# andyljones/megastep

Hardware: AMD Instinct MI355X
Metric: env-steps/sec (higher is better)
Workload: dtype f32

## Files before the change

megastep_amd/_lib.py:

```python
import ctypes as C
import os
import subprocess
import torch

_HERE = os.path.dirname(os.path.abspath(__file__))
CSRC = os.path.join(_HERE, 'csrc')
LIB_PATH = os.environ.get('MEGASTEP_HIP_LIB') or os.path.join(CSRC, 'libmegastep_hip.so')
ABI_VERSION = 17

_f32p = C.POINTER(C.c_float)
_i32p = C.POINTER(C.c_int)


class MsConfig(C.Structure):
    _fields_ = [('agent_radius', C.c_float), ('res', C.c_int), ('fov', C.c_float), ('fps', C.c_float)]


class MsScenery(C.Structure):
    _fields_ = [
        ('n_envs', C.c_int), ('n_agents', C.c_int), ('n_model', C.c_int),
        ('lights_vals', C.c_void_p), ('lights_widths', C.c_void_p), ('lights_starts', C.c_void_p),
        ('lines_vals', C.c_void_p), ('lines_widths', C.c_void_p), ('lines_starts', C.c_void_p),
        ('lines_inverse', C.c_void_p),
        ('textures_vals', C.c_void_p), ('textures_widths', C.c_void_p), ('textures_starts', C.c_void_p),
# ... 139 lines not shown
    'ms_overhead': (_int, [_p(MsScenery), _p(MsAgents), _p(MsOverhead), _ptr]),
    'ms_nav_free': (_int, [_p(MsScenery), _p(MsNavGrid), _ptr]),
    'ms_nav_fields': (_int, [_p(MsNavGrid), _p(MsNavFields), _ptr]),
    'ms_nav_query': (_int, [_p(MsNavGrid), _p(MsNavQuery), _ptr]),
    'ms_nav_waypoints': (_int, [_p(MsNavGrid), _p(MsNavWaypoints), _ptr]),
    'ms_nav_paths': (_int, [_p(MsNavGrid), _p(MsNavPaths), _ptr]),
    'ms_nav_seen': (_int, [_p(MsNavGrid), _p(MsNavSeen), _ptr]),
    'ms_nav_windows': (_int, [_p(MsNavGrid), _p(MsNavWindows), _ptr]),
    'ms_nav_seed_fields': (_int, [_p(MsNavGrid), _p(MsNavSeedFields), _ptr]),
    'ms_nav_seed_waypoints': (_int, [_p(MsNavGrid), _p(MsNavSeedWaypoints), _ptr]),
    'ms_nav_seed_paths': (_int, [_p(MsNavGrid), _p(MsNavSeedPaths), _ptr]),
    'ms_wallgrid_scan': (_int, [_p(MsScenery), _p(MsWallGridParent), _ptr, _int, _int, _ptr, _ptr, _ptr, _ptr]),
    'ms_wallgrid_fill': (_int, [_p(MsScenery), _ptr, _int, _int, _ptr, _ptr, _ptr, _ptr, _ptr, _ptr]),
    'ms_host_ray_interval': (None, [_f32p, _f32p, _int, _flt, _flt, _int, _i32p, _i32p]),
    'ms_host_ray_interval_wide': (None, [_f32p, _f32p, _int, _flt, _flt, _int, _int, _i32p, _i32p]),
    'ms_debug_ray_groups': (_int, [_int]),
    'ms_debug_physics_pack': (_int, [_int]),
    'ms_debug_last_render_groups': (_int, []),
    'ms_debug_last_step_fused': (_int, []),
    'ms_host_render_plan': (C.c_longlong, [_int, _int, _int, _int, _int, _flt, _int, _i32p]),
    'ms_host_render_block': (_int, [_int, _int, _int, _int, _int, _flt, _int, C.c_longlong, _i32p]),
    'ms_host_physics_pack': (_int, [_int, _int, _int, _int]),
    'ms_debug_render_order': (_int, [_int]),
    'ms_host_order_fans': (_int, [_int, _i32p, _i32p]),
    'ms_debug_ray_group_tail': (_int, [_flt, _int]),
    'ms_debug_pair_telemetry': (_int, [_int]),
    'ms_debug_overhead_cull': (_int, [_int]),
    'ms_host_overhead_keeps': (_int, [_f32p, _int, _int, _int, _int, _flt, _f32p]),
    'ms_host_nav_waypoint': (_int, [_ptr, _flt, _ptr, _ptr, _ptr, _ptr, _int, _ptr]),
    'ms_host_nav_path': (_int, [_ptr, _flt, _ptr, _ptr, _ptr, _ptr, _int, _ptr]),
    'ms_host_nav_seed_field': (_int, [_ptr, _flt, _ptr, _ptr, _int, _ptr, _int, _ptr, _ptr]),
    'ms_host_nav_seed_waypoint': (_int, [_ptr, _flt, _ptr, _ptr, _ptr, _int, _ptr]),
    'ms_host_nav_seed_path': (_int, [_ptr, _flt, _ptr, _ptr, _ptr, _int, _ptr]),
    'ms_host_nav_seen': (_int, [_ptr, _flt, _ptr, _int, _int, _int, _ptr, _ptr, _ptr, _ptr, _flt, _ptr, _ptr, _ptr, _ptr]),
    'ms_host_nav_windows': (_int, [_p(MsNavGrid), _p(MsNavWindows)]),
    'ms_test_arithmetic': (_int, [_ptr]*7 + [C.c_longlong, _ptr]),
    'ms_host_lightgrid_cell': (_int, [_ptr, _int, _ptr, _int, _flt, _flt, _int, _int, _flt, _int, _ptr, _ptr, _int]),
    'ms_host_fold_hits': (_int, [_f32p, _i32p, _int, _i32p, _f32p, _i32p]),
    'ms_host_agents_apart': (_int, [_f32p, _f32p, _flt]),
    'ms_host_wall_beyond_reach': (_int, [_f32p, _f32p, _flt]),
    'ms_host_wall_reach': (_flt, [_f32p, _flt]),
    'ms_host_wall_hidden': (_int, [_flt]*4 + [_f32p, _f32p, _flt]),
    'ms_host_wall_sectors': (None, [_flt]*4 + [_f32p, _i32p, _i32p, _f32p, _i32p]),
    'ms_host_wallgrid_cell': (None, [_ptr, _int, _flt, _flt, _int, _int, _flt, _int, _flt, _flt, _flt, _ptr, _ptr]),
    'ms_host_wall_arc': (None, [_flt]*4 + [_f32p, _i32p, _i32p]),
    'ms_host_wedge_meets': (_int, [_flt]*4 + [_int, _int]),
# ... 100 lines not shown
```

megastep_amd/csrc/kernels/render.h:

```cpp
constexpr int PAIRS = 128;

struct Cand { float pqx, pqy, vx, vy; };

__device__ __attribute__((noinline)) float2 sincospi_called(const float x) {
    float s_, c_;
    sincospi_f(x, s_, c_);
    return make_float2(s_, c_);
}

__device__ inline float4 drawn_row(const float s, const float c, const float px, const float py, const float4 mdl) {
    float4 w;
    w.x = c*mdl.x - s*mdl.y + px; w.y = s*mdl.x + c*mdl.y + py;
    w.z = c*mdl.z - s*mdl.w + px; w.w = s*mdl.z + c*mdl.w + py;
    return w;
}
__device__ inline void camera_ray(const float cs, const float sn, const int r, const float Rf, const float half_screen,
                                  const float inv_res, float& rx, float& ry) {
    const float num = (Rf - 2*(float)r - 1)*half_screen;
    const float uy = inv_res != 0.f ? num*inv_res : div_inrange(num, Rf);
    rx = cs*1.f - sn*uy; ry = sn*1.f + cs*uy;
}
__host__ inline float camera_inv_res(const int R, const float half_screen) {
    return ((R & (R - 1)) == 0 && half_screen > 1e-3f) ? 1.f/(float)R : 0.f;
}
// ... 209 lines not shown
#define MS_AHEAD 1
#endif
#ifndef MS_VCAP
#define MS_VCAP 128
#endif
#ifndef MS_VCAP_WIDE
#define MS_VCAP_WIDE 110
#endif
#ifndef MS_WAVES_WIDE
#define MS_WAVES_WIDE 6
#endif
template <int OBS, int SHADE = 1, int NG = 1, int STEP = 0>
__global__ __launch_bounds__(WAVE) __attribute__((amdgpu_waves_per_eu(NG > 1 ? MS_WAVES_WIDE : MS_WAVES, NG > 1 ? MS_WAVES_WIDE : MS_WAVES))) void render_kernel(
        const MsScenery sc, const AgentsK ag, const MsRender out,
        const float agent_radius, const float half_screen, const int R, const int n_fans,
        const std::conditional_t<STEP == 1, RenderConstsStep, std::conditional_t<NG == 1, RenderConstsOrder, RenderConsts>> rc) {
    static_assert(STEP == 0 || NG == 1, "the fused step: one group of rays");
    constexpr bool ORDERED = NG == 1 && STEP == 0;
    PROBE_INIT
    static_assert(NG == 1 || NG == 2 || NG == 4, "one, two or four ray groups per wave");
    [[maybe_unused]] constexpr int NR = WAVE*NG;
    constexpr int VCAP = NG == 1 ? MS_VCAP : MS_VCAP_WIDE;
    constexpr int O_EPI = NG > 1 ? 24*VCAP + 256 : 0;
    constexpr int LDS_PER_WAVE = NG == 1 ? 24*VCAP + 3072 : O_EPI + 2816 + 6*VCAP;
    __shared__ __attribute__((aligned(16))) unsigned char s_raw[LDS_PER_WAVE];

    int lane = threadIdx.x;
#define LANE_AFRESH asm volatile("" : "+v"(lane))
    Cand* const s_cand_w = reinterpret_cast<Cand*>(&s_raw[0]);
    float* const s_screen_w = reinterpret_cast<float*>(&s_raw[O_EPI]);

    const int b = blockIdx.x;
    [[maybe_unused]] int fan = b;
    const int A = sc.n_agents, AF = sc.n_agents*sc.n_model;
    int n, a, r0, span;
    if constexpr (ORDERED) {
        const int slot = render_slot(b, n_fans);
        const int* const at = rc.schedule ? rc.schedule + n_fans + slot : sc.lines_starts;
        const int named = *at;
        fan = rc.schedule ? (int)min((unsigned)named, (unsigned)(n_fans - 1)) : slot;
        render_fan(fan, A, R, rc, n, a, r0, span);
    } else if (!render_block(b, n_fans, A, R, NG, rc, n, a, r0, span, fan)) return;
    const int r = r0 + lane;
    const int r_last = min(r0 + span - 1, R - 1);
    [[maybe_unused]] const int n_live = r_last - r0 + 1;

    const int L = sc.lines_widths[n];
// ... 177 lines not shown
    const float Rf = (float)R;
    auto ray_len = [&](const float rx_, const float ry_) {
        return sqrt_normal(rx_*rx_ + ry_*ry_);
    };
    auto ray_of = [&](const int r_, float& rx_, float& ry_, float& rlen_, float& near_) {
        camera_ray(cs, sn, r_, Rf, half_screen, rc.inv_res, rx_, ry_);
        rlen_ = ray_len(rx_, ry_);
        near_ = div_inrange(agent_radius, rlen_);
    };
    float rx, ry, rlen, near;
    ray_of(r, rx, ry, rlen, near);

    const float c_a = 0.5f*(Rf - 1.f), c_b = rc.c_b;
    const float x_clip = rc.x_clip;
    const float g0 = (float)r0;

    constexpr bool COLOUR = SHADE != 0;
    static_assert(COLOUR || OBS == 1, "without colour `screen` is NULL: the OBS instantiation");
    static_assert(OBS != 2 || (COLOUR && STEP == 0), "no per-ray planes at all: a colour instantiation");
    constexpr bool PLANES = OBS != 2;
    constexpr bool MASKED = !COLOUR || (OBS >= 1 && NG == 1);
    [[maybe_unused]] const int out_mask_ = MASKED ? (out.obs_subsample >> 8) : 0;
#define MS_WANTED(BIT, PTR) (MASKED ? ((out_mask_ & (BIT)) != 0) : ((PTR) != nullptr))
    [[maybe_unused]] int fan_cost = 0;
    auto winner_of = [&](const int nearest_idx, float4& hw_mem, int& tex_w, int& tstart) {
        const LateArgs late = late_args();
        const bool want_texel_row = COLOUR || (OBS && MS_WANTED(OUT_SEEN, late->out.seen_stamp));
        const bool want_line = want_texel_row || MS_WANTED(OUT_LOCATIONS, late->out.locations) || MS_WANTED(OUT_DOTS, late->out.dots);
        const int row = min(max(nearest_idx, 0), max(L - 1, 0));
        hw_mem = make_float4(0.f, 0.f, 0.f, 0.f); tex_w = 1; tstart = 0;
        if (want_line) hw_mem = rows.row(row);
        if (want_texel_row) {
            const int* const l_tex_widths = late->sc.textures_widths;
            const int* const l_tex_starts = late->sc.textures_starts;
            tex_w = l_tex_widths[base + row]; tstart = l_tex_starts[base + row];
        }
    };
    auto finish_group = [&](const int q, const int r, const float rx, const float ry, const float rlen,
                            const float nearest_s, const int nearest_idx, const float4 hw_mem, const int tex_w, const int tstart) {
    const LateArgs late = late_args();
    const bool want_texel_row = COLOUR || (OBS && MS_WANTED(OUT_SEEN, late->out.seen_stamp));
    const bool want_line = want_texel_row || MS_WANTED(OUT_LOCATIONS, late->out.locations) || MS_WANTED(OUT_DOTS, late->out.dots);
    float loc = NAN, dt = NAN;
    float4 hw = make_float4(0.f, 0.f, 0.f, 0.f);
    if (want_line) {
        float4 aw = make_float4(0.f, 0.f, 0.f, 0.f);
        if (__ballot((nearest_idx >= 0) & (nearest_idx < AF))) aw = agent_line(nearest_idx);
        if (nearest_idx >= 0) {
            hw = (nearest_idx < AF) ? aw : hw_mem;
            const float vx = hw.z - hw.x, vy = hw.w - hw.y;
            const float d = rx*vy - ry*vx;
            const float pqx = hw.x - pp.x, pqy = hw.y - pp.y;
            loc = div_inrange(pqx*ry - pqy*rx, d);
            const float dtop = rx*vx + ry*vy;
            const float dbot = rlen*sqrt_any(vx*vx + vy*vy);
            dt = div_inrange(dtop, dbot + 1.e-6f);
        }
    }
    [[maybe_unused]] const size_t o = ((size_t)n*A + a)*R + r;
    const float dist = nearest_s*rlen;
    if constexpr (PLANES) {
        if (!MASKED || (out_mask_ & (OUT_INDICES | OUT_LOCATIONS | OUT_DOTS | OUT_DISTANCES))) {
            int* const o_indices = late->out.indices;
            float* const o_locations = late->out.locations;
            float* const o_dots = late->out.dots;
            float* const o_distances = late->out.distances;
            if (r < R) {
                if (!OBS || MS_WANTED(OUT_INDICES, o_indices)) __builtin_nontemporal_store(nearest_idx, &o_indices[o]);
                if (!OBS || MS_WANTED(OUT_LOCATIONS, o_locations)) __builtin_nontemporal_store(loc, &o_locations[o]);
                if (!OBS || MS_WANTED(OUT_DOTS, o_dots)) __builtin_nontemporal_store(dt, &o_dots[o]);
                if (!OBS || MS_WANTED(OUT_DISTANCES, o_distances)) __builtin_nontemporal_store(dist, &o_distances[o]);
            }
        }
    }

// ... 120 lines not shown
        }
        for (int o2 = 4; o2 < sub; o2 <<= 1) {
            if constexpr (COLOUR) {
                p0 += __shfl_xor(p0, o2, WAVE); p1 += __shfl_xor(p1, o2, WAVE); p2 += __shfl_xor(p2, o2, WAVE);
            }
            pd += __shfl_xor(pd, o2, WAVE);
        }
        if (((lane & (sub - 1)) == 0) & (r < R)) {
            const int sh = __builtin_ctz((unsigned)sub);
            const float inv = bits_f((uint32_t)(127 - sh) << 23);
            const int W = R >> sh, px = r >> sh;
            const size_t na = (size_t)n*A + a;
            if (COLOUR && MS_WANTED(OUT_RGB, late->out.obs_rgb)) {
                late->out.obs_rgb[(na*3 + 0)*W + px] = p0*inv;
                late->out.obs_rgb[(na*3 + 1)*W + px] = p1*inv;
                late->out.obs_rgb[(na*3 + 2)*W + px] = p2*inv;
            }
            if (MS_WANTED(OUT_DEPTH, late->out.obs_depth)) late->out.obs_depth[na*W + px] = pd*inv;
        }
    }
    };
    float nearest_s = INFINITY;
    int nearest_idx = -1;

    constexpr int V_CAP = VCAP, P_CAP = 4096 < 64*VCAP ? 4096 : 64*VCAP;
    constexpr int O_INFO = 16*V_CAP;
    constexpr int O_QUEUE = NG == 1 ? 24*V_CAP + 768 : 24*V_CAP;
    constexpr int O_RAY = NG == 1 ? 24*V_CAP : O_EPI, O_NEAR = O_RAY + 512, O_BEST = NG == 1 ? O_QUEUE + 256 : O_NEAR + 256;
    constexpr int O_MARK = O_BEST + 1536, O_PINFO = O_MARK + 512, O_GK = O_PINFO + 4*V_CAP;
    static_assert((NG == 1 ? O_MARK + 512 : O_GK + 2*V_CAP) == LDS_PER_WAVE && LDS_PER_WAVE >= 2560, "the LDS block: lists, rays, queue, three key slots, 4096 mark bits");
    static_assert(NG == 1 || O_EPI + 2560 <= LDS_PER_WAVE, "the epilogue's scratch fits the per-group region");
    int2* const s_info_w = reinterpret_cast<int2*>(&s_raw[O_INFO]);
    float2* const s_ray_w = reinterpret_cast<float2*>(&s_raw[O_RAY]);
    float* const s_near_w = reinterpret_cast<float*>(&s_raw[O_NEAR]);
    unsigned long long* const s_best_w = reinterpret_cast<unsigned long long*>(&s_raw[O_BEST]);
    unsigned long long* const s_second_w = reinterpret_cast<unsigned long long*>(&s_raw[O_BEST + 512]);
    unsigned long long* const s_third_w = reinterpret_cast<unsigned long long*>(&s_raw[O_BEST + 1024]);
    unsigned* const s_mark_w = reinterpret_cast<unsigned*>(&s_raw[O_MARK]);
    if constexpr (NG == 1) {
        s_ray_w[lane] = make_float2(rx, ry);
        s_near_w[lane] = near;
        s_best_w[lane] = ~0ull;
        s_mark_w[lane] = 0u; s_mark_w[lane + WAVE] = 0u;
        s_second_w[lane] = ~0ull;
        s_third_w[lane] = ~0ull;
    }
    auto pseudo_angle_fast = [](const float x_, const float y_) {
        const float pq_ = y_*__builtin_amdgcn_rcpf(fabsf(x_) + fabsf(y_));
        return x_ < 0.f ? 2.f - pq_ : (pq_ < 0.f ? 4.f + pq_ : pq_);
    };
    const float pa_first = readlane_f(pseudo_angle_fast(rx, ry), 0);
    float pa_last = readlane_f(pseudo_angle_fast(rx, ry), min(n_live, WAVE) - 1);
    float sp_g0 = g0, sp_last = (float)(r_last - r0), sp_nr = (float)WAVE;
    auto fetch = [&](const int c0) { return rows.chunk(lane, c0); };
    auto line_math = [&](float4 w, const int l, const bool live, const bool agent_lines, const bool first_chunk, Cand& cd, int& lo, int& len) {
        if (agent_lines) {
            const float4 aw = agent_line_m(l, first_chunk, mdl_first);
            if (l < AF) w = aw;
        }
        const float pqx = w.x - pp.x, pqy = w.y - pp.y;
        const float dbx = w.z - pp.x, dby = w.w - pp.y;
// ... 39 lines not shown
                if (beyond) {
                    const unsigned long long key = ((unsigned long long)f_bits(sv) << 32) | (unsigned)info.y;
                    const unsigned long long old = atomicMin(&s_best_w[rr], key);
                    const unsigned oh = (unsigned)(old >> 32);
                    if (oh != 0xffffffffu) {
                        const bool won = key < old;
                        const float so = bits_f(oh);
                        const float front = won ? sv : so, back = won ? so : sv;
                        if (back < front + 4.e-4f) {
                            const unsigned long long lose1 = won ? old : key;
                            const unsigned long long old2 = atomicMin(&s_second_w[rr], lose1);
                            const unsigned long long lose2 = old2 > lose1 ? old2 : lose1;
                            if (lose2 != ~0ull) atomicMin(&s_third_w[rr], lose2);
                        }
                    }
                }
            }
        }
        __builtin_amdgcn_wave_barrier();
        s_mark_w[lane] = 0u; s_mark_w[lane + WAVE] = 0u;
        n_list = 0; n_pairs = 0;
    };

    auto admit = [&](const float4 w, const int l, const bool live, const bool agent_lines, const bool first_chunk) {
        Cand cd;
        int lo = 0, len = 0;
        line_math(w, l, live, agent_lines, first_chunk, cd, lo, len);
        const bool seen = len > 0;
        const unsigned long long vm = __ballot(seen);
        if (!vm) return;
        const int incl = wave_scan_add(len);
        const int chunk_pairs = __builtin_amdgcn_readlane(incl, 63);
        const int chunk_lines = __popcll(vm);
        if ((n_list + chunk_lines > V_CAP) | (n_pairs + chunk_pairs > P_CAP)) drain();
        if (seen) {
            const int k = n_list + (int)__builtin_amdgcn_mbcnt_hi((unsigned)(vm >> 32), __builtin_amdgcn_mbcnt_lo((unsigned)vm, 0u));
            const int first = n_pairs + incl - len;
            s_cand_w[k] = cd;
            s_info_w[k] = make_int2(lo - first, l);
            atomicOr(&s_mark_w[first >> 5], 1u << (first & 31));
        }
        n_list += chunk_lines; n_pairs += chunk_pairs;
    };

    constexpr int Q_CAP = 128;
    unsigned short* const s_queue_w = reinterpret_cast<unsigned short*>(&s_raw[O_QUEUE]);
    const bool listed = wg_count >= 0;
    const int n_raw = listed ? wg_count : max(L - AF, 0);
    const int own0 = a*sc.n_model, own = rc.skip_own ? sc.n_model : 0;
    const int AL = AF - own;
    const __amdgpu_buffer_rsrc_t list_rsrc = __builtin_amdgcn_make_buffer_rsrc(
        const_cast<unsigned*>(sc.wg_pool + wg_pool_base_n + wg_first), 0, listed ? 4*n_raw : 0, 0x00020000);
    auto raw = [&](const int k0) {
        return (unsigned)__builtin_amdgcn_raw_buffer_load_b32(list_rsrc, 4*(k0 + lane), 0, 0);
    };
    auto walk = [&](const float pa_right, const float pa_left, auto&& admit_fn, auto&& stop_fn) {
        int wa8, wb8;
        wg_wedge(pa_right, pa_left, wa8, wb8);
        unsigned e_next[2] = {raw(0), raw(WAVE)};
        int raw_pos = 0, q_len = 0, al_left = AL;
        int q_first = 0;
        for (;;) {
            while ((raw_pos < n_raw) & (q_len <= Q_CAP - WAVE)) {
                const unsigned e = e_next[0];
                e_next[0] = e_next[1];
                e_next[1] = raw(raw_pos + 2*WAVE);
                const int k = raw_pos + lane;
                const int idx = listed ? (int)(e & 0xffffu) : k;
                const bool keep = (k < n_raw) & (!listed | wg_arcs_meet((int)((e >> 16) & 255u), (int)(e >> 24), wa8, wb8));
                const unsigned long long km = __ballot(keep);
                if (keep) s_queue_w[q_len + (int)__builtin_amdgcn_mbcnt_hi((unsigned)(km >> 32), __builtin_amdgcn_mbcnt_lo((unsigned)km, 0u))] = (unsigned short)idx;
                q_len += __popcll(km);
                raw_pos += WAVE;
            }
            __builtin_amdgcn_fence(__ATOMIC_RELEASE, "wavefront");
            __builtin_amdgcn_wave_barrier();
            __builtin_amdgcn_fence(__ATOMIC_ACQUIRE, "wavefront");
            const int al0 = AL - al_left;
            const int n_al = min(al_left, AHEAD*WAVE);
            const int n_items = n_al + min(q_len, AHEAD*WAVE - n_al);
            const int q_used = n_items - n_al;
            int l_it[AHEAD];
            float4 w_it[AHEAD];
            #pragma unroll
            for (int kk = 0; kk < AHEAD; kk++) {
                const int i = kk*WAVE + lane;
                const int ai = al0 + i;
                const int q_at = min(max(i - n_al, 0), Q_CAP - 1);
                const int qe = listed ? (int)s_queue_w[q_at] : q_first + q_at;
                l_it[kk] = (i < n_al) ? ai + (ai >= own0 ? own : 0) : AF + qe;
                w_it[kk] = rows.load(l_it[kk]*16, 0);
            }
            PROBE_VAL(2, 0)
            PROBE_AT(3, w_it[0].x)
            #pragma unroll
            for (int kk = 0; kk < AHEAD; kk++) {
                if (kk*WAVE >= n_items) continue;
                admit_fn(w_it[kk], l_it[kk], kk*WAVE + lane < n_items, kk*WAVE < n_al, al0 + kk*WAVE == 0);
            }
            al_left -= n_al;
            __builtin_amdgcn_wave_barrier();
            if (q_used < q_len) {
                unsigned short keep_[Q_CAP/WAVE];
                #pragma unroll
                for (int j = 0; j < Q_CAP/WAVE; j++) keep_[j] = s_queue_w[min(q_used + j*WAVE + lane, Q_CAP - 1)];
                __builtin_amdgcn_wave_barrier();
                #pragma unroll
                for (int j = 0; j < Q_CAP/WAVE; j++) if (j*WAVE + lane < q_len - q_used) s_queue_w[j*WAVE + lane] = keep_[j];
            }
            q_len -= q_used;
            q_first += q_used;
            if (((raw_pos >= n_raw) & (q_len == 0) & (al_left == 0)) || stop_fn()) break;
        }
    };
    if constexpr (NG == 1) {
        walk(pa_last, pa_first, admit, [] { return false; });
        if (n_pairs) drain();
    }
    __builtin_amdgcn_fence(__ATOMIC_ACQUIRE, "wavefront");
    bool list_whole = true;
    auto resolve_group = [&](const int q, const float rx, const float ry, const float near, float& nearest_s, int& nearest_idx) {
        const unsigned long long best = s_best_w[lane], second = s_second_w[lane], third = s_third_w[lane];
        bool ambiguous = false;
        if (best != ~0ull) {
            const float s1 = bits_f((uint32_t)(best >> 32)), s2 = bits_f((uint32_t)(second >> 32)), s3 = bits_f((uint32_t)(third >> 32));
            const int i1 = (int)(uint32_t)best, i2 = (int)(uint32_t)second;
            nearest_s = s1;
            nearest_idx = i1;
            if ((second != ~0ull) && !(s1 < s2 - 1.e-4f)) {
                if ((third == ~0ull) || (s2 < s3 - 1.e-4f)) {
                    const bool first_is_1 = i1 < i2;
                    const float sa = first_is_1 ? s1 : s2, sb = first_is_1 ? s2 : s1;
                    const int ia = first_is_1 ? i1 : i2, ib = first_is_1 ? i2 : i1;
                    const bool b_wins = sb < sa - 1.e-4f;
                    nearest_s = b_wins ? sb : sa;
                    nearest_idx = b_wins ? ib : ia;
                } else {
                    ambiguous = true;
                }
            }
        }
        const unsigned long long amb = __ballot(ambiguous);
        if constexpr (ORDERED) fan_cost = n_windows + (list_n >> 5) + 4*(int)__popcll(amb);
        PROBE_VAL(11, n_pairs_total) PROBE_VAL(12, n_drains == 1 ? list_n : -1) PROBE_VAL(13, __popcll(amb))
#if MS_PROBE
        const unsigned t_fold0 = (unsigned)clock64();
        PROBE_VAL(15, t_fold0)
#endif
        if (out.workspace && lane == 0 && q == 0 && rc.telemetry) {
            atomicAdd(&out.workspace[3], n_pairs_total); atomicAdd(&out.workspace[4], n_windows);
        }
        if (amb && out.workspace && lane == 0) {
            atomicAdd(&out.workspace[1], __popcll(amb));
            if (__popcll(amb) > 6) atomicAdd(&out.workspace[2], 1);
        }
        if (amb && (NG == 1 ? n_drains == 1 : list_whole)) {
            const int rounds = (list_n + WAVE - 1)/WAVE;
            if (2*(int)__popcll(amb)*rounds <= list_n + 16) {
                float x = INFINITY;
                int xi = -1;
                for (int k0 = 0; k0 < list_n; k0 += WAVE) {
                    const int k = min(k0 + lane, list_n - 1);
                    const Cand cd = s_cand_w[k];
                    const int line = s_info_w[k].y;
                    const float cpv = cd.pqx*cd.vy - cd.pqy*cd.vx;
                    for (unsigned long long todo = amb; todo; todo &= todo - 1) {
                        const int jr = __ffsll((long long)todo) - 1;
                        const float jrx = readlane_f(rx, jr), jry = readlane_f(ry, jr), jnear = readlane_f(near, jr);
                        const float d = jrx*cd.vy - jry*cd.vx;
                        const float nt = cd.pqx*jry - cd.pqy*jrx;
                        const float ad = fabsf(d);
                        const float ntp = bits_f(f_bits(nt) ^ (f_bits(d) & 0x80000000u));
                        bool valid = false;
                        float sv = 0.f;
                        if ((k0 + lane < list_n) & (ad >= 1.e-3f) & (ntp >= 0.f) & (ntp <= ad)) {
                            sv = div_inrange(cpv, d);
                            valid = jnear < sv;
                        }
                        unsigned long long m = __ballot(valid);
                        if (m) {
                            float xs = readlane_f(x, jr);
                            int xis = __builtin_amdgcn_readlane(xi, jr);
                            for (; m; m &= m - 1) {
                                const int j = __ffsll((long long)m) - 1;
                                const float sj = readlane_f(sv, j);
                                if (sj < xs - 1.e-4f) { xs = sj; xis = __builtin_amdgcn_readlane(line, j); }
                            }
                            if (lane == jr) { x = xs; xi = xis; }
                        }
                    }
                }
                if (ambiguous) { nearest_s = x; nearest_idx = xi; }
            } else {
                float x = INFINITY;
                int xi = -1;
                #pragma unroll 4
                for (int k = 0; k < list_n; k++) {
                    const Cand cd = s_cand_w[k];
                    const int line = s_info_w[k].y;
                    if (ambiguous) {
                        const float d = rx*cd.vy - ry*cd.vx;
                        const float nt = cd.pqx*ry - cd.pqy*rx;
                        const float ad = fabsf(d);
                        const float ntp = bits_f(f_bits(nt) ^ (f_bits(d) & 0x80000000u));
                        if ((ad >= 1.e-3f) & (ntp >= 0.f) & (ntp <= ad)) {
                            const float sv = div_inrange(cd.pqx*cd.vy - cd.pqy*cd.vx, d);
                            if ((near < sv) & (sv < x - 1.e-4f)) { x = sv; xi = line; }
                        }
                    }
                }
                if (ambiguous) { nearest_s = x; nearest_idx = xi; }
            }
        } else
        if (__popcll(amb) > 6) {
            float x = INFINITY;
            int xi = -1;
            for (int c0 = 0; c0 < L; c0 += WAVE) {
                Cand mine;
                int lo = 0, len = 0;
                line_math(fetch(c0), c0 + lane, c0 + lane < L, c0 < AF, NG == 1 && c0 == 0, mine, lo, len);
                __builtin_amdgcn_wave_barrier();
                s_cand_w[lane] = mine;
// ... 44 lines not shown
                    bool valid = false;
                    float sv = 0.f;
                    if ((l < L) & (ad >= 1.e-3f) & (ntp >= 0.f) & (ntp <= ad)) {
                        sv = div_inrange(pqx*vy - pqy*vx, d);
                        valid = jnear < sv;
                    }
                    unsigned long long m = __ballot(valid);
                    if (m) {
                        float xs = readlane_f(x, jr);
                        int xis = __builtin_amdgcn_readlane(xi, jr);
                        for (; m; m &= m - 1) {
                            const int j = __ffsll((long long)m) - 1;
                            const float sj = readlane_f(sv, j);
                            if (sj < xs - 1.e-4f) { xs = sj; xis = c0 + j; }
                        }
                        if (lane == jr) { x = xs; xi = xis; }
                    }
                }
            }
            if (ambiguous) { nearest_s = x; nearest_idx = xi; }
        }
    };
    if constexpr (NG == 1) {
        resolve_group(0, rx, ry, near, nearest_s, nearest_idx);
    } else {
        int* const s_pinfo_w = reinterpret_cast<int*>(&s_raw[O_PINFO]);
        unsigned short* const s_gk_w = reinterpret_cast<unsigned short*>(&s_raw[O_GK]);
        const int n_groups = (n_live + WAVE - 1)/WAVE;
        auto pass2_group = [&](const int lo_g) {
            __builtin_amdgcn_fence(__ATOMIC_RELEASE, "wavefront");
            __builtin_amdgcn_wave_barrier();
            __builtin_amdgcn_fence(__ATOMIC_ACQUIRE, "wavefront");
            int base = 0, nj = 0;
            auto windows = [&]() {
                __builtin_amdgcn_fence(__ATOMIC_RELEASE, "wavefront");
                __builtin_amdgcn_wave_barrier();
                __builtin_amdgcn_fence(__ATOMIC_ACQUIRE, "wavefront");
                n_pairs_total += base; n_windows += (base + WAVE - 1)/WAVE;
                const unsigned long long my_marks = reinterpret_cast<const unsigned long long*>(s_mark_w)[lane];
                int before = 0;
                for (int p0 = 0; p0 < base; p0 += WAVE) {
                    const unsigned mlo = (unsigned)__builtin_amdgcn_readlane((int)(unsigned)my_marks, p0 >> 6);
                    const unsigned mhi = (unsigned)__builtin_amdgcn_readlane((int)(unsigned)(my_marks >> 32), p0 >> 6);
                    const unsigned long long M = ((unsigned long long)mhi << 32) | mlo;
                    const unsigned long long Ms = M >> 1;
                    const int upto = (int)(mlo & 1u) + (int)__builtin_amdgcn_mbcnt_hi((unsigned)(Ms >> 32), __builtin_amdgcn_mbcnt_lo((unsigned)Ms, 0u));
                    const int p = p0 + lane;
// ... 58 lines not shown
            if (base) windows();
        };
        auto setup_group = [&](const int q, float& qx, float& qy, float& ql, float& qn) {
            ray_of(r0 + q*WAVE + lane, qx, qy, ql, qn);
            __builtin_amdgcn_wave_barrier();
            s_ray_w[lane] = make_float2(qx, qy);
            s_near_w[lane] = qn;
            s_best_w[lane] = ~0ull; s_second_w[lane] = ~0ull; s_third_w[lane] = ~0ull;
            s_mark_w[lane] = 0u; s_mark_w[lane + WAVE] = 0u;
        };
        auto span_of = [&](const int q0, const int sp_n) {
            const int sp_rays = min(n_live - q0*WAVE, sp_n*WAVE);
            sp_g0 = (float)(r0 + q0*WAVE); sp_last = (float)(sp_rays - 1); sp_nr = (float)(sp_n*WAVE);
            float wx, wy, wl_, wn_;
            ray_of(r0 + q0*WAVE + (lane == 0 ? 0 : sp_rays - 1), wx, wy, wl_, wn_);
            return pseudo_angle_fast(wx, wy);
        };
        auto group_rest = [&](const int q, const int q_rel, const float gx, const float gy) {
            pass2_group(q_rel*WAVE);
            list_n = n_list;
            __builtin_amdgcn_fence(__ATOMIC_ACQUIRE, "wavefront");
            float ns = INFINITY;
            int ni = -1;
            resolve_group(q_rel, gx, gy, s_near_w[lane], ns, ni);
            LANE_AFRESH;
            float4 hw_mem; int tex_w, tstart;
            winner_of(ni, hw_mem, tex_w, tstart);
            finish_group(q, r0 + q*WAVE + lane, gx, gy, ray_len(gx, gy), ns, ni, hw_mem, tex_w, tstart);
            __builtin_amdgcn_wave_barrier();
        };
        bool overflow = false;
        {
            const float pa = span_of(0, n_groups);
            n_list = 0; list_whole = true;
            auto admit_shared = [&](const float4 w, const int l, const bool live, const bool agent_lines, const bool) {
                if (overflow) return;
                Cand cd;
                int lo = 0, len = 0;
                line_math(w, l, live, agent_lines, false, cd, lo, len);
                const bool seen = len > 0;
                const unsigned long long vm = __ballot(seen);
                if (!vm) return;
                const int chunk_lines = __popcll(vm);
                if (n_list + chunk_lines > V_CAP) { overflow = true; return; }
                if (seen) {
                    const int k = n_list + (int)__builtin_amdgcn_mbcnt_hi((unsigned)(vm >> 32), __builtin_amdgcn_mbcnt_lo((unsigned)vm, 0u));
                    s_cand_w[k] = cd;
                    s_info_w[k] = make_int2(lo | (len << 16), l);
                }
                n_list += chunk_lines;
            };
            walk(readlane_f(pa, 1), readlane_f(pa, 0), admit_shared, [&] { return overflow; });
        }
        if (!overflow) {
            #pragma unroll 1
            for (int q = 0; q < n_groups; q++) {
                LANE_AFRESH;
                if (q) load_agents();
                float gx, gy, gl, gn;
                setup_group(q, gx, gy, gl, gn);
                group_rest(q, q, gx, gy);
            }
        } else {
            #pragma unroll 1
            for (int q = 0; q < n_groups; q++) {
                LANE_AFRESH;
                if (q) load_agents();
                const float pa = span_of(q, 1);
                float gx, gy, gl, gn;
                setup_group(q, gx, gy, gl, gn);
                n_list = 0; list_whole = true;
                auto admit_one = [&](const float4 w, const int l, const bool live, const bool agent_lines, const bool) {
                    Cand cd;
                    int lo = 0, len = 0;
                    line_math(w, l, live, agent_lines, false, cd, lo, len);
                    const bool seen = len > 0;
                    const unsigned long long vm = __ballot(seen);
                    if (!vm) return;
                    const int chunk_lines = __popcll(vm);
                    if (n_list + chunk_lines > V_CAP) {
                        pass2_group(0);
                        n_list = 0; list_whole = false;
                    }
                    if (seen) {
                        const int k = n_list + (int)__builtin_amdgcn_mbcnt_hi((unsigned)(vm >> 32), __builtin_amdgcn_mbcnt_lo((unsigned)vm, 0u));
                        s_cand_w[k] = cd;
                        s_info_w[k] = make_int2(lo | (len << 16), l);
                    }
                    n_list += chunk_lines;
                };
                walk(readlane_f(pa, 1), readlane_f(pa, 0), admit_one, [] { return false; });
                const float2 back = s_ray_w[lane];
                group_rest(q, 0, back.x, back.y);
            }
        }
    }

    PROBE_AT(4, nearest_idx)
    if constexpr (NG == 1) {
        float4 hw_mem; int tex_w, tstart;
        winner_of(nearest_idx, hw_mem, tex_w, tstart);
        finish_group(0, r, rx, ry, rlen, nearest_s, nearest_idx, hw_mem, tex_w, tstart);
    }
    PROBE_DONE(fan)
#undef MS_WANTED
}


__global__ __launch_bounds__(WG) void dynlight_kernel(
        const MsScenery sc, const AgentsK ag, const MsRender out, const int R) {
    __shared__ LightPair s_pair[WAVES][PAIRS];
    __shared__ unsigned s_shadow[2*WAVE];

    const int tid = threadIdx.x, wave = tid >> 6, lane = tid & 63;
    int fan = blockIdx.x;
    if (out.workspace) {
        if (fan >= out.workspace[0]) return;
        fan = out.workspace[16 + fan];
    }
    const int A = sc.n_agents, AF = sc.n_agents*sc.n_model;
    const int G = (R + WAVE - 1)/WAVE, F = A*G;
    const int n = fan / F, rem = fan - n*F, a = rem / G, g = rem - a*G;
    const int r = g*WAVE + lane;
    const size_t o = ((size_t)n*A + a)*R + r;
    const int L = sc.lines_widths[n];
// ... 149 lines not shown
```

megastep_amd/csrc/megastep_hip.hip:

```cpp
#include <hip/hip_runtime.h>
#include <math.h>
#include <stdint.h>
#include <stddef.h>
#include <stdlib.h>
#include <string.h>
#include <atomic>
#include <vector>
#include "../../include/megastep_hip_test.h"

namespace {

constexpr float AMBIENT = .1f;
constexpr float LUMINANCE = 2.f;
constexpr int WAVE = 64;
constexpr int WG = 256;
constexpr int WAVES = WG/WAVE;

thread_local int g_last_hip_error = 0;
thread_local int g_pair_telemetry = 0;
thread_local int g_ray_groups = 0;
thread_local int g_physics_pack = 0;
thread_local float g_tail_rounds = -1.f;
thread_local int g_tail_envs = -1;
thread_local int g_last_step_fused = 0;
thread_local int g_last_render_groups = 0;
thread_local int g_overhead_cull = 1;
thread_local int g_render_order = 1;

struct AgentsK { float* angles; float* positions; float* angvelocity; float* velocity; float* headings; };
AgentsK agents_k(const MsAgents& a) { return AgentsK{a.angles, a.positions, a.angvelocity, a.velocity, a.headings}; }

#ifndef MS_PROBE
#define MS_PROBE 0
#endif
#if MS_PROBE
constexpr int PROBE_STAMPS = 8;
constexpr int PROBE_WORDS = 16;
__device__ unsigned* g_probe = nullptr;
__device__ long long g_probe_cap = 0;
struct Probe {
    unsigned t = 0u, real0 = (unsigned)wall_clock64();
    __device__ void done(const int lane, const long long wave) {
        if (g_probe && wave < g_probe_cap) {
            unsigned v = t;
            if (lane == PROBE_STAMPS) v = ((unsigned)__builtin_amdgcn_s_getreg((31 << 11) | 4) & 0xffffu) | ((unsigned)(__builtin_amdgcn_s_getreg((3 << 11) | 20) & 0xf) << 16);
            if (lane == PROBE_STAMPS + 1) v = real0;
            if (lane == PROBE_STAMPS + 2) v = (unsigned)wall_clock64();
            if (lane < PROBE_WORDS) g_probe[wave*PROBE_WORDS + lane] = v;
        }
    }
// ... 154 lines not shown
}
#endif

int ms_debug_ray_groups(int groups) { g_ray_groups = groups; return MS_OK; }
int ms_debug_last_render_groups(void) { return g_last_render_groups; }
int ms_debug_physics_pack(int envs) { g_physics_pack = envs; return MS_OK; }
int ms_host_physics_pack(int n_envs, int n_agents, int gridded, int pinned) { return physics_pack_of(n_envs, n_agents, gridded != 0, pinned); }
long long ms_host_render_plan(int n_envs, int n_agents, int res, int slots, int pinned_groups, float tail_rounds, int tail_envs, int* groups) {
    RenderConsts rc;
    const RenderPlan plan = render_plan(n_envs, n_agents, res, slots, pinned_groups, tail_rounds, tail_envs, rc);
    if (groups) *groups = plan.ng;
    return plan.n_blocks;
}
int ms_host_render_block(int n_envs, int n_agents, int res, int slots, int pinned_groups, float tail_rounds, int tail_envs, long long block, int* out4) {
    RenderConsts rc;
    const RenderPlan plan = render_plan(n_envs, n_agents, res, slots, pinned_groups, tail_rounds, tail_envs, rc);
    int fan = 0;
    if (block < 0 || block >= plan.n_blocks) return -1;
    return render_block((int)block, (int)plan.n_blocks, n_agents, res, plan.ng, rc, out4[0], out4[1], out4[2], out4[3], fan) ? 1 : 0;
}
int ms_debug_ray_group_tail(float rounds, int envs) { g_tail_rounds = rounds; g_tail_envs = envs; return MS_OK; }
int ms_debug_pair_telemetry(int on) { g_pair_telemetry = on ? 1 : 0; return MS_OK; }
int ms_debug_render_order(int on) { g_render_order = on ? 1 : 0; return MS_OK; }
int ms_host_order_fans(int n_fans, const int* costs, int* order) {
    if (n_fans < 1 || !costs || !order) return -1;
    const int K = fan_sort_per_run(n_fans);
    for (int block = 0; block < 8*K; block++) {
        int first_fan, count, first_slot, next[FAN_CLASSES] = {0};
        fan_sort_part(n_fans, K, block, first_fan, count, first_slot);
        for (int i = 0; i < count; i++) next[fan_class(costs[first_fan + i])]++;
        for (int c = FAN_CLASSES - 1, rank = 0; c >= 0; c--) { const int m = next[c]; next[c] = rank; rank += m; }
        for (int i = 0; i < count; i++) order[first_slot + K*next[fan_class(costs[first_fan + i])]++] = first_fan + i;
    }
    return 8*K;
}

int ms_test_arithmetic(const float* n, const float* d, float* q_inrange, float* q_ieee, const float* x, float* r_any, float* r_ieee,
                       long long count, void* stream) {
    if (count < 0 || ((q_inrange || q_ieee) && !(n && d)) || ((r_any || r_ieee) && !x)) return MS_EINVAL;
    if (count == 0) return MS_OK;
    const long long blocks = (count + WG - 1)/WG;
    if (blocks > 0x7fffffffLL) return MS_EUNSUPPORTED;
    hipLaunchKernelGGL(arithmetic_test_kernel, dim3((unsigned)blocks), dim3(WG), 0, (hipStream_t)stream, n, d, q_inrange, q_ieee, x, r_any, r_ieee, count);
    return launch_status();
}

// ... 235 lines not shown
    const bool pooled = out->obs_rgb || out->obs_depth || out->obs_centre || out->seen_stamp;
    if (L.dynlight && (!all_planes || pooled)) return MS_EUNSUPPORTED;
    if (!pooled && !out->indices && !out->locations && !out->dots && !out->distances && !out->screen) return MS_EINVAL;
    L.obs = pooled || !all_planes;
    L.no_planes = L.colour && !out->indices && !out->locations && !out->dots && !out->distances && !out->screen;
    const bool physics_listed = sc->wg_cells != nullptr;
    L.fused = progress && sc->n_agents == 1 && R <= WAVE && L.plan.ng == 1 && physics_listed == L.walls_listed &&
              (!physics_listed || (sc->wg_near_rows && (uintptr_t)sc->wg_near_rows % 16 == 0));
    const bool cached = ag->headings && !L.dynlight;
    L.prep = !cached && !L.fused && out->workspace;
    if ((cached && (uintptr_t)ag->headings % 16) || (L.prep && (uintptr_t)out->workspace % 8)) return MS_EINVAL;
    L.agn = agents_k(*ag);
    L.outn = *out;
    L.schedule = (schedule_serves(ag, sc, R) && L.plan.ng == 1 && !L.fused) ? ag->schedule : nullptr;
    if (L.schedule && (uintptr_t)L.schedule % 4) return MS_EINVAL;
    if (!cached && !L.fused) L.agn.headings = nullptr;
    if (!L.prep) L.outn.workspace = nullptr;
    if (out->obs_depth) L.outn.obs_max_depth = 1.f/out->obs_max_depth;
    L.rc.x_clip = 0.5f*cfg->agent_radius/sqrtf(1.f + half_screen*half_screen);
    L.rc.c_b = 0.5f*(float)R/half_screen;
    L.rc.by_m = divisor_of((unsigned)sc->n_model);
    L.rc.skip_own = (sc->model_radius > 0.f && sc->model_radius*1.01f < cfg->agent_radius) ? 1 : 0;
    L.rc.inv_res = camera_inv_res(R, half_screen);
    L.rc.telemetry = g_pair_telemetry;
    if (!L.colour || (L.obs && L.plan.ng == 1))
        L.outn.obs_subsample = (out->obs_subsample & 0xff) | (((out->indices ? OUT_INDICES : 0) | (out->locations ? OUT_LOCATIONS : 0) |
                                (out->dots ? OUT_DOTS : 0) | (out->distances ? OUT_DISTANCES : 0) | (out->obs_depth ? OUT_DEPTH : 0) |
                                (out->obs_centre ? OUT_CENTRE : 0) | (out->seen_stamp ? OUT_SEEN : 0) | (out->screen ? OUT_SCREEN : 0) |
                                (out->obs_rgb ? OUT_RGB : 0)) << 8);
    if (L.fused) {
        L.rc.progress = progress; L.rc.fps = cfg->fps; L.rc.wg_cells_physics = sc->wg_cells;
        step_options_of(mv, ex, L.rc.mv, L.rc.ex);
    }
    return MS_OK;
}

static int render_enqueue(const RenderLaunch& L, const hipStream_t hs) {
    g_last_render_groups = L.plan.ng;
    const int na = L.scn.n_envs*L.scn.n_agents;
    if (L.prep) hipLaunchKernelGGL(render_prep_kernel, dim3((na + WG - 1)/WG), dim3(WG), 0, hs, agents_k(*L.ag), L.out->workspace, na, L.rc.ws_headings);
    RenderConstsOrder rco;
    static_cast<RenderConsts&>(rco) = L.rc; rco.schedule = L.schedule;
#define MS_LAUNCH_RENDER(O, S, NG_, STEP_) hipLaunchKernelGGL((render_kernel<O, S, NG_, STEP_>), dim3((int)L.plan.n_blocks), dim3(WAVE), 0, hs, \
                                                              L.scn, L.agn, L.outn, L.agent_radius, L.half_screen, L.R, (int)L.plan.n_blocks, L.rc)
#define MS_LAUNCH_RENDER_OS(NG_) { if (!L.colour) MS_LAUNCH_RENDER(1, 0, NG_, 0); else if (L.no_planes) MS_LAUNCH_RENDER(2, 1, NG_, 0); \
                                   else if (L.obs) MS_LAUNCH_RENDER(1, 1, NG_, 0); else MS_LAUNCH_RENDER(0, 1, NG_, 0); }
    if (L.fused) { if (!L.colour) MS_LAUNCH_RENDER(1, 0, 1, 1); else if (L.obs) MS_LAUNCH_RENDER(1, 1, 1, 1); else MS_LAUNCH_RENDER(0, 1, 1, 1); }
// ... 442 lines not shown
```

megastep_amd/cuda.py:

```python
import ctypes as C
import numbers
import os
import torch
from . import _call, _lib, grids
from ._lib import _on, _stream
from ._call import _agents_on, _cfg, _check, _require_gpu, config

_switched = __import__('threading').local()


def _ab_switches():
    if getattr(_switched, 'done', False):
        return
    _switched.done = True
    g = os.environ.get('MEGASTEP_RAY_GROUPS')
    if g:
        _lib.lib().ms_debug_ray_groups(int(g))
    k = os.environ.get('MEGASTEP_PHYSICS_PACK')
    if k:
        _lib.lib().ms_debug_physics_pack(int(k))
    o = os.environ.get('MEGASTEP_RENDER_ORDER')
    if o:
        _lib.lib().ms_debug_render_order(int(o))
    t, e = os.environ.get('MEGASTEP_RAY_GROUP_TAIL'), os.environ.get('MEGASTEP_RAY_GROUP_TAIL_ENVS')
    if t or e:
        _lib.lib().ms_debug_ray_group_tail(float(t) if t else -1., int(e) if e else -1)


def initialize(agent_radius, res, fov, fps):
    _call._config = config(agent_radius, res, fov, fps)
    _ab_switches()


class _Ragged:
    _ndim = None

    def __init__(self, vals, widths):
        _check(vals, 'vals', torch.float32, self._ndim)
        _check(widths, 'widths', torch.int32, 1)
        if vals.device != widths.device:
            raise RuntimeError('vals and widths must be on the same device')
        ends = widths.cumsum(0).to(torch.int32)
        total = int(ends[-1]) if len(widths) else 0
        if total != vals.shape[0]:
            raise RuntimeError(f'widths sum to {total} but vals has {vals.shape[0]} rows')
        self._vals, self._widths = vals, widths
# ... 478 lines not shown
```

Before: 106.1 million.

## Reuse LDS candidate list for winner line and texture rows in render epilogue

```diff
diff --git a/megastep_amd/_lib.py b/megastep_amd/_lib.py
--- a/megastep_amd/_lib.py
+++ b/megastep_amd/_lib.py
@@ -185,6 +185,7 @@
     'ms_host_render_block': (_int, [_int, _int, _int, _int, _int, _flt, _int, C.c_longlong, _i32p]),
     'ms_host_physics_pack': (_int, [_int, _int, _int, _int]),
     'ms_debug_render_order': (_int, [_int]),
+    'ms_debug_winner_rows': (_int, [_int]),
     'ms_host_order_fans': (_int, [_int, _i32p, _i32p]),
     'ms_debug_ray_group_tail': (_int, [_flt, _int]),
     'ms_debug_pair_telemetry': (_int, [_int]),
diff --git a/megastep_amd/csrc/kernels/render.h b/megastep_amd/csrc/kernels/render.h
--- a/megastep_amd/csrc/kernels/render.h
+++ b/megastep_amd/csrc/kernels/render.h
@@ -255,7 +255,8 @@
     [[maybe_unused]] constexpr int NR = WAVE*NG;
     constexpr int VCAP = NG == 1 ? MS_VCAP : MS_VCAP_WIDE;
     constexpr int O_EPI = NG > 1 ? 24*VCAP + 256 : 0;
-    constexpr int LDS_PER_WAVE = NG == 1 ? 24*VCAP + 3072 : O_EPI + 2816 + 6*VCAP;
+    constexpr bool WROWS = NG == 1 && (SHADE != 0 || STEP == 0);
+    constexpr int LDS_PER_WAVE = NG == 1 ? (WROWS ? 26 : 24)*VCAP + 3072 : O_EPI + 2816 + 6*VCAP;
     __shared__ __attribute__((aligned(16))) unsigned char s_raw[LDS_PER_WAVE];
 
     int lane = threadIdx.x;
@@ -479,22 +480,45 @@
     constexpr bool MASKED = !COLOUR || (OBS >= 1 && NG == 1);
     [[maybe_unused]] const int out_mask_ = MASKED ? (out.obs_subsample >> 8) : 0;
 #define MS_WANTED(BIT, PTR) (MASKED ? ((out_mask_ & (BIT)) != 0) : ((PTR) != nullptr))
+    [[maybe_unused]] const bool wrows = WROWS && (rc.telemetry & 2) != 0;
+    [[maybe_unused]] const int kshift = wrows ? 7 : 0;
+    [[maybe_unused]] const bool want_tex_p1 = COLOUR || (OBS && (out_mask_ & OUT_SEEN) != 0);
     [[maybe_unused]] int fan_cost = 0;
-    auto winner_of = [&](const int nearest_idx, float4& hw_mem, int& tex_w, int& tstart) {
+    auto winner_of = [&](const int nearest_idx, [[maybe_unused]] const int win_k, [[maybe_unused]] const bool drained_once, float4& hw_mem, bool& from_list, int& tex_w, int& tstart) {
         const LateArgs late = late_args();
         const bool want_texel_row = COLOUR || (OBS && MS_WANTED(OUT_SEEN, late->out.seen_stamp));
         const bool want_line = want_texel_row || MS_WANTED(OUT_LOCATIONS, late->out.locations) || MS_WANTED(OUT_DOTS, late->out.dots);
         const int row = min(max(nearest_idx, 0), max(L - 1, 0));
-        hw_mem = make_float4(0.f, 0.f, 0.f, 0.f); tex_w = 1; tstart = 0;
-        if (want_line) hw_mem = rows.row(row);
-        if (want_texel_row) {
-            const int* const l_tex_widths = late->sc.textures_widths;
-            const int* const l_tex_starts = late->sc.textures_starts;
-            tex_w = l_tex_widths[base + row]; tstart = l_tex_starts[base + row];
+        hw_mem = make_float4(0.f, 0.f, 0.f, 0.f); tex_w = 1; tstart = 0; from_list = false;
+        bool ask = true;
+        if constexpr (WROWS) {
+            if (wrows & drained_once & want_line) {
+                const int k = win_k & 127;
+                const Cand cd = s_cand_w[k];
+                const unsigned ix = (unsigned)reinterpret_cast<const int2*>(&s_raw[16*VCAP])[k].x;
+                const unsigned ax = reinterpret_cast<const unsigned short*>(&s_raw[LDS_PER_WAVE - 2*VCAP])[k];
+                const bool ok = (win_k >= 0) & (!want_texel_row | ((ax >> 5) != 0u));
+                if (ok) {
+                    hw_mem = make_float4(cd.pqx, cd.pqy, cd.vx, cd.vy); from_list = true;
+                    if (want_texel_row) { tex_w = (int)(ax >> 5); tstart = (int)((ix >> 6) | ((ax & 31u) << 26)); }
+                }
+                ask = (nearest_idx >= 0) & !ok;
+            }
+        }
+        if (__ballot(ask)) {
+            float4 hw_ = make_float4(0.f, 0.f, 0.f, 0.f); int tw_ = 1, ts_ = 0;
+            if (want_line) hw_ = rows.row(row);
+            if (want_texel_row) {
+                const int* const l_tex_widths = late->sc.textures_widths;
+                const int* const l_tex_starts = late->sc.textures_starts;
+                tw_ = l_tex_widths[base + row]; ts_ = l_tex_starts[base + row];
+            }
+            if (ask) { hw_mem.x = hw_.x; hw_mem.y = hw_.y; hw_mem.z = hw_.z; hw_mem.w = hw_.w; tex_w = tw_; tstart = ts_; }
         }
     };
     auto finish_group = [&](const int q, const int r, const float rx, const float ry, const float rlen,
-                            const float nearest_s, const int nearest_idx, const float4 hw_mem, const int tex_w, const int tstart) {
+                            const float nearest_s, const int nearest_idx, const float4 hw_mem, [[maybe_unused]] const bool from_list,
+                            const int tex_w, const int tstart) {
     const LateArgs late = late_args();
     const bool want_texel_row = COLOUR || (OBS && MS_WANTED(OUT_SEEN, late->out.seen_stamp));
     const bool want_line = want_texel_row || MS_WANTED(OUT_LOCATIONS, late->out.locations) || MS_WANTED(OUT_DOTS, late->out.dots);
@@ -505,9 +529,12 @@
         if (__ballot((nearest_idx >= 0) & (nearest_idx < AF))) aw = agent_line(nearest_idx);
         if (nearest_idx >= 0) {
             hw = (nearest_idx < AF) ? aw : hw_mem;
-            const float vx = hw.z - hw.x, vy = hw.w - hw.y;
+            float vx = hw.z - hw.x, vy = hw.w - hw.y;
+            float pqx = hw.x - pp.x, pqy = hw.y - pp.y;
+            if constexpr (WROWS) {
+                if (from_list & (nearest_idx >= AF)) { pqx = hw_mem.x; pqy = hw_mem.y; vx = hw_mem.z; vy = hw_mem.w; }
+            }
             const float d = rx*vy - ry*vx;
-            const float pqx = hw.x - pp.x, pqy = hw.y - pp.y;
             loc = div_inrange(pqx*ry - pqy*rx, d);
             const float dtop = rx*vx + ry*vy;
             const float dbot = rlen*sqrt_any(vx*vx + vy*vy);
@@ -674,13 +701,16 @@
     };
     float nearest_s = INFINITY;
     int nearest_idx = -1;
+    [[maybe_unused]] int win_k = -1;
 
     constexpr int V_CAP = VCAP, P_CAP = 4096 < 64*VCAP ? 4096 : 64*VCAP;
     constexpr int O_INFO = 16*V_CAP;
     constexpr int O_QUEUE = NG == 1 ? 24*V_CAP + 768 : 24*V_CAP;
     constexpr int O_RAY = NG == 1 ? 24*V_CAP : O_EPI, O_NEAR = O_RAY + 512, O_BEST = NG == 1 ? O_QUEUE + 256 : O_NEAR + 256;
     constexpr int O_MARK = O_BEST + 1536, O_PINFO = O_MARK + 512, O_GK = O_PINFO + 4*V_CAP;
-    static_assert((NG == 1 ? O_MARK + 512 : O_GK + 2*V_CAP) == LDS_PER_WAVE && LDS_PER_WAVE >= 2560, "the LDS block: lists, rays, queue, three key slots, 4096 mark bits");
+    constexpr int O_AUX = O_MARK + 512;
+    static_assert(!WROWS || (V_CAP <= 128 && LDS_PER_WAVE <= 6400 && O_INFO == 16*VCAP && O_AUX == LDS_PER_WAVE - 2*VCAP), "a slot is seven bits of a key; five LDS granules a wave");
+    static_assert((NG == 1 ? O_AUX + (WROWS ? 2*V_CAP : 0) : O_GK + 2*V_CAP) == LDS_PER_WAVE && LDS_PER_WAVE >= 2560, "the LDS block: lists, rays, queue, three key slots, 4096 mark bits");
     static_assert(NG == 1 || O_EPI + 2560 <= LDS_PER_WAVE, "the epilogue's scratch fits the per-group region");
     int2* const s_info_w = reinterpret_cast<int2*>(&s_raw[O_INFO]);
     float2* const s_ray_w = reinterpret_cast<float2*>(&s_raw[O_RAY]);
@@ -689,6 +719,7 @@
     unsigned long long* const s_second_w = reinterpret_cast<unsigned long long*>(&s_raw[O_BEST + 512]);
     unsigned long long* const s_third_w = reinterpret_cast<unsigned long long*>(&s_raw[O_BEST + 1024]);
     unsigned* const s_mark_w = reinterpret_cast<unsigned*>(&s_raw[O_MARK]);
+    [[maybe_unused]] unsigned short* const s_aux_w = reinterpret_cast<unsigned short*>(&s_raw[WROWS ? O_AUX : 0]);
     if constexpr (NG == 1) {
         s_ray_w[lane] = make_float2(rx, ry);
         s_near_w[lane] = near;
@@ -774,7 +805,8 @@
         n_list = 0; n_pairs = 0;
     };
 
-    auto admit = [&](const float4 w, const int l, const bool live, const bool agent_lines, const bool first_chunk) {
+    auto admit = [&](const float4 w, const int l, const bool live, const bool agent_lines, const bool first_chunk,
+                     [[maybe_unused]] const int tw, [[maybe_unused]] const int ts) {
         Cand cd;
         int lo = 0, len = 0;
         line_math(w, l, live, agent_lines, first_chunk, cd, lo, len);
@@ -789,7 +821,15 @@
             const int k = n_list + (int)__builtin_amdgcn_mbcnt_hi((unsigned)(vm >> 32), __builtin_amdgcn_mbcnt_lo((unsigned)vm, 0u));
             const int first = n_pairs + incl - len;
             s_cand_w[k] = cd;
-            s_info_w[k] = make_int2(lo - first, l);
+            int ix = lo - first, ly = l;
+            if constexpr (WROWS) {
+                if (wrows) {
+                    ix = (ix & 63) | (int)((unsigned)ts << 6);
+                    ly = (l << 7) | k;
+                    s_aux_w[k] = (unsigned short)(((unsigned)ts >> 26) | (((tw >= 1) & (tw <= 2047)) ? (unsigned)tw << 5 : 0u));
+                }
+            }
+            s_info_w[k] = make_int2(ix, ly);
             atomicOr(&s_mark_w[first >> 5], 1u << (first & 31));
         }
         n_list += chunk_lines; n_pairs += chunk_pairs;
@@ -834,6 +874,7 @@
             const int q_used = n_items - n_al;
             int l_it[AHEAD];
             float4 w_it[AHEAD];
+            [[maybe_unused]] int tw_it[AHEAD], ts_it[AHEAD];
             #pragma unroll
             for (int kk = 0; kk < AHEAD; kk++) {
                 const int i = kk*WAVE + lane;
@@ -843,12 +884,23 @@
                 l_it[kk] = (i < n_al) ? ai + (ai >= own0 ? own : 0) : AF + qe;
                 w_it[kk] = rows.load(l_it[kk]*16, 0);
             }
+            if constexpr (WROWS) {
+                #pragma unroll
+                for (int kk = 0; kk < AHEAD; kk++) {
+                    tw_it[kk] = 0; ts_it[kk] = 0;
+                    if (want_tex_p1) {
+                        const int row_c = base + min(l_it[kk], max(L - 1, 0));
+                        tw_it[kk] = sc.textures_widths[row_c]; ts_it[kk] = sc.textures_starts[row_c];
+                    }
+                }
+            }
             PROBE_VAL(2, 0)
             PROBE_AT(3, w_it[0].x)
             #pragma unroll
             for (int kk = 0; kk < AHEAD; kk++) {
                 if (kk*WAVE >= n_items) continue;
-                admit_fn(w_it[kk], l_it[kk], kk*WAVE + lane < n_items, kk*WAVE < n_al, al0 + kk*WAVE == 0);
+                if constexpr (WROWS) admit_fn(w_it[kk], l_it[kk], kk*WAVE + lane < n_items, kk*WAVE < n_al, al0 + kk*WAVE == 0, tw_it[kk], ts_it[kk]);
+                else admit_fn(w_it[kk], l_it[kk], kk*WAVE + lane < n_items, kk*WAVE < n_al, al0 + kk*WAVE == 0, 0, 0);
             }
             al_left -= n_al;
             __builtin_amdgcn_wave_barrier();
@@ -871,7 +923,8 @@
     }
     __builtin_amdgcn_fence(__ATOMIC_ACQUIRE, "wavefront");
     bool list_whole = true;
-    auto resolve_group = [&](const int q, const float rx, const float ry, const float near, float& nearest_s, int& nearest_idx) {
+    auto resolve_group = [&](const int q, const float rx, const float ry, const float near, float& nearest_s, int& nearest_idx,
+                             [[maybe_unused]] int& win_k) {
         const unsigned long long best = s_best_w[lane], second = s_second_w[lane], third = s_third_w[lane];
         bool ambiguous = false;
         if (best != ~0ull) {
@@ -892,6 +945,10 @@
                 }
             }
         }
+        if constexpr (WROWS) {
+            win_k = (wrows & (nearest_idx >= 0) & !ambiguous) ? (nearest_idx & 127) : -1;
+            nearest_idx >>= kshift;
+        }
         const unsigned long long amb = __ballot(ambiguous);
         if constexpr (ORDERED) fan_cost = n_windows + (list_n >> 5) + 4*(int)__popcll(amb);
         PROBE_VAL(11, n_pairs_total) PROBE_VAL(12, n_drains == 1 ? list_n : -1) PROBE_VAL(13, __popcll(amb))
@@ -899,7 +956,7 @@
         const unsigned t_fold0 = (unsigned)clock64();
         PROBE_VAL(15, t_fold0)
 #endif
-        if (out.workspace && lane == 0 && q == 0 && rc.telemetry) {
+        if (out.workspace && lane == 0 && q == 0 && (rc.telemetry & 1)) {
             atomicAdd(&out.workspace[3], n_pairs_total); atomicAdd(&out.workspace[4], n_windows);
         }
         if (amb && out.workspace && lane == 0) {
@@ -914,7 +971,7 @@
                 for (int k0 = 0; k0 < list_n; k0 += WAVE) {
                     const int k = min(k0 + lane, list_n - 1);
                     const Cand cd = s_cand_w[k];
-                    const int line = s_info_w[k].y;
+                    const int line = s_info_w[k].y >> kshift;
                     const float cpv = cd.pqx*cd.vy - cd.pqy*cd.vx;
                     for (unsigned long long todo = amb; todo; todo &= todo - 1) {
                         const int jr = __ffsll((long long)todo) - 1;
@@ -949,7 +1006,7 @@
                 #pragma unroll 4
                 for (int k = 0; k < list_n; k++) {
                     const Cand cd = s_cand_w[k];
-                    const int line = s_info_w[k].y;
+                    const int line = s_info_w[k].y >> kshift;
                     if (ambiguous) {
                         const float d = rx*cd.vy - ry*cd.vx;
                         const float nt = cd.pqx*ry - cd.pqy*rx;
@@ -1040,7 +1097,7 @@
         }
     };
     if constexpr (NG == 1) {
-        resolve_group(0, rx, ry, near, nearest_s, nearest_idx);
+        resolve_group(0, rx, ry, near, nearest_s, nearest_idx, win_k);
     } else {
         int* const s_pinfo_w = reinterpret_cast<int*>(&s_raw[O_PINFO]);
         unsigned short* const s_gk_w = reinterpret_cast<unsigned short*>(&s_raw[O_GK]);
@@ -1145,18 +1202,20 @@
             __builtin_amdgcn_fence(__ATOMIC_ACQUIRE, "wavefront");
             float ns = INFINITY;
             int ni = -1;
-            resolve_group(q_rel, gx, gy, s_near_w[lane], ns, ni);
+            int no_k = -1;
+            resolve_group(q_rel, gx, gy, s_near_w[lane], ns, ni, no_k);
             LANE_AFRESH;
             float4 hw_mem; int tex_w, tstart;
-            winner_of(ni, hw_mem, tex_w, tstart);
-            finish_group(q, r0 + q*WAVE + lane, gx, gy, ray_len(gx, gy), ns, ni, hw_mem, tex_w, tstart);
+            bool from_list;
+            winner_of(ni, -1, false, hw_mem, from_list, tex_w, tstart);
+            finish_group(q, r0 + q*WAVE + lane, gx, gy, ray_len(gx, gy), ns, ni, hw_mem, false, tex_w, tstart);
             __builtin_amdgcn_wave_barrier();
         };
         bool overflow = false;
         {
             const float pa = span_of(0, n_groups);
             n_list = 0; list_whole = true;
-            auto admit_shared = [&](const float4 w, const int l, const bool live, const bool agent_lines, const bool) {
+            auto admit_shared = [&](const float4 w, const int l, const bool live, const bool agent_lines, const bool, const int, const int) {
                 if (overflow) return;
                 Cand cd;
                 int lo = 0, len = 0;
@@ -1193,7 +1252,7 @@
                 float gx, gy, gl, gn;
                 setup_group(q, gx, gy, gl, gn);
                 n_list = 0; list_whole = true;
-                auto admit_one = [&](const float4 w, const int l, const bool live, const bool agent_lines, const bool) {
+                auto admit_one = [&](const float4 w, const int l, const bool live, const bool agent_lines, const bool, const int, const int) {
                     Cand cd;
                     int lo = 0, len = 0;
                     line_math(w, l, live, agent_lines, false, cd, lo, len);
@@ -1222,8 +1281,9 @@
     PROBE_AT(4, nearest_idx)
     if constexpr (NG == 1) {
         float4 hw_mem; int tex_w, tstart;
-        winner_of(nearest_idx, hw_mem, tex_w, tstart);
-        finish_group(0, r, rx, ry, rlen, nearest_s, nearest_idx, hw_mem, tex_w, tstart);
+        bool from_list;
+        winner_of(nearest_idx, win_k, n_drains == 1, hw_mem, from_list, tex_w, tstart);
+        finish_group(0, r, rx, ry, rlen, nearest_s, nearest_idx, hw_mem, from_list, tex_w, tstart);
     }
     PROBE_DONE(fan)
 #undef MS_WANTED
diff --git a/megastep_amd/csrc/megastep_hip.hip b/megastep_amd/csrc/megastep_hip.hip
--- a/megastep_amd/csrc/megastep_hip.hip
+++ b/megastep_amd/csrc/megastep_hip.hip
@@ -26,6 +26,7 @@
 thread_local int g_last_render_groups = 0;
 thread_local int g_overhead_cull = 1;
 thread_local int g_render_order = 1;
+thread_local int g_winner_rows = 1;
 
 struct AgentsK { float* angles; float* positions; float* angvelocity; float* velocity; float* headings; };
 AgentsK agents_k(const MsAgents& a) { return AgentsK{a.angles, a.positions, a.angvelocity, a.velocity, a.headings}; }
@@ -226,6 +227,7 @@
 int ms_debug_ray_group_tail(float rounds, int envs) { g_tail_rounds = rounds; g_tail_envs = envs; return MS_OK; }
 int ms_debug_pair_telemetry(int on) { g_pair_telemetry = on ? 1 : 0; return MS_OK; }
 int ms_debug_render_order(int on) { g_render_order = on ? 1 : 0; return MS_OK; }
+int ms_debug_winner_rows(int on) { g_winner_rows = on ? 1 : 0; return MS_OK; }
 int ms_host_order_fans(int n_fans, const int* costs, int* order) {
     if (n_fans < 1 || !costs || !order) return -1;
     const int K = fan_sort_per_run(n_fans);
@@ -507,7 +509,7 @@
     L.rc.by_m = divisor_of((unsigned)sc->n_model);
     L.rc.skip_own = (sc->model_radius > 0.f && sc->model_radius*1.01f < cfg->agent_radius) ? 1 : 0;
     L.rc.inv_res = camera_inv_res(R, half_screen);
-    L.rc.telemetry = g_pair_telemetry;
+    L.rc.telemetry = (g_pair_telemetry ? 1 : 0) | ((g_winner_rows && sc->n_lines_total <= (1 << 24)) ? 2 : 0);
     if (!L.colour || (L.obs && L.plan.ng == 1))
         L.outn.obs_subsample = (out->obs_subsample & 0xff) | (((out->indices ? OUT_INDICES : 0) | (out->locations ? OUT_LOCATIONS : 0) |
                                 (out->dots ? OUT_DOTS : 0) | (out->distances ? OUT_DISTANCES : 0) | (out->obs_depth ? OUT_DEPTH : 0) |
diff --git a/megastep_amd/cuda.py b/megastep_amd/cuda.py
--- a/megastep_amd/cuda.py
+++ b/megastep_amd/cuda.py
@@ -22,6 +22,9 @@
     o = os.environ.get('MEGASTEP_RENDER_ORDER')
     if o:
         _lib.lib().ms_debug_render_order(int(o))
+    w = os.environ.get('MEGASTEP_WINNER_ROWS')
+    if w:
+        _lib.lib().ms_debug_winner_rows(int(w))
     t, e = os.environ.get('MEGASTEP_RAY_GROUP_TAIL'), os.environ.get('MEGASTEP_RAY_GROUP_TAIL_ENVS')
     if t or e:
         _lib.lib().ms_debug_ray_group_tail(float(t) if t else -1., int(e) if e else -1)
```

New measurement: 104.5 million. 0.985x the previous value.
